# conroi/lcpc

Hardware: AMD Instinct MI355X
Metric: field-elements committed/sec (whole node), Ligero 2^26 coeffs (higher is better)
Workload: dtype u32 limbs (255-bit prime field Ft255, Montgomery form)

## Files before the change

### lcpc_amd/csrc/field_ln.h

```cpp
#pragma once
#include "field_dev.h"

namespace lcpc {

template <int NL, int W> constexpr u32 mod_limb(int k) {
  const int b = W * k, w = b / 32, sh = b % 32;
  const u64 lo = Mod<NL>::P[w], hi = (w + 1 < NL) ? Mod<NL>::P[w + 1] : 0;
  return (u32)(((lo | (hi << 32)) >> sh) & ((1u << W) - 1));
}
template <int FID> struct LnField;
template <> struct LnField<FT63> {
  static constexpr int FID = FT63, N = 3, W = 26, NL = 2, WAVES = 8, STRIDE = 4;
  static constexpr u32 limb(int k) { return mod_limb<NL, W>(k); }
};
template <> struct LnField<FT127> {
  static constexpr int FID = FT127, N = 5, W = 29, NL = 4, WAVES = 7, STRIDE = 8;
  static constexpr u32 limb(int k) { return mod_limb<NL, W>(k); }
};
template <> struct LnField<FT191> {
  static constexpr int FID = FT191, N = 7, W = 29, NL = 6, WAVES = 5, STRIDE = 8;
  static constexpr u32 limb(int k) { return mod_limb<NL, W>(k); }
};
template <> struct LnField<FT255> {
  static constexpr int FID = FT255, N = 9, W = 29, NL = 8, WAVES = 4, STRIDE = 12;
  static constexpr u32 limb(int k) { return mod_limb<NL, W>(k); }
};

#include "field_ln_gen.h"
#include "field_r29_gen.h"
#include "field_wmul_gen.h"

template <int N> struct LN {
  u32 v[N];
};

namespace ln {
constexpr int QOFF = 24;
constexpr int QBIAS = 40;

template <class FT> LCPC_DEV LN<FT::N> from_packed(const Fe<FT::NL>& a) {
  constexpr int N = FT::N, W = FT::W, NL = FT::NL;
  LN<N> r;
#pragma unroll
  for (int k = 0; k < N; k++) {
    const int b = W * k, w = b / 32, sh = b % 32;
    u32 x;
    if (sh == 0) x = a.v[w];
    else if (w + 1 < NL) x = __builtin_amdgcn_alignbit(a.v[w + 1], a.v[w], sh);
    else x = a.v[w] >> sh;
    r.v[k] = k + 1 < N ? (x & ((1u << W) - 1)) : x;
  }
  return r;
}
template <class FT> LCPC_DEV void to_packed(u32* out, const u32* l) {
  constexpr int N = FT::N, W = FT::W, NL = FT::NL;
#pragma unroll
  for (int w = 0; w < NL; w++) {
    u32 x = 0;
#pragma unroll
    for (int k = 0; k < N; k++) {
      const int off = W * k - 32 * w;
      if (off >= 0 && off < 32) x |= l[k] << off;
      else if (off < 0 && off > -32) x |= l[k] >> (-off);
    }
    out[w] = x;
  }
}
template <int N> LCPC_DEV LN<N> load_limbs(const u32* t) {
  LN<N> r;
  if constexpr (N == 3) {
    const uint2 a = *reinterpret_cast<const uint2*>(t);
    r.v[0] = a.x; r.v[1] = a.y; r.v[2] = t[2];
  } else {
    const uint4 a = *reinterpret_cast<const uint4*>(t);
    r.v[0] = a.x; r.v[1] = a.y; r.v[2] = a.z; r.v[3] = a.w;
    if constexpr (N == 5) r.v[4] = t[4];
    else if constexpr (N == 7) { const uint2 b = *reinterpret_cast<const uint2*>(t + 4); r.v[4] = b.x; r.v[5] = b.y; r.v[6] = t[6]; }
    else { const uint4 b = *reinterpret_cast<const uint4*>(t + 4); r.v[4] = b.x; r.v[5] = b.y; r.v[6] = b.z; r.v[7] = b.w; r.v[8] = t[8]; }
  }
  return r;
}
template <int N> LCPC_DEV LN<N> add(const LN<N>& a, const LN<N>& b) {
  LN<N> r;
#pragma unroll
  for (int k = 0; k < N; k++) r.v[k] = a.v[k] + b.v[k];
  return r;
}
template <int N> LCPC_DEV LN<N> sub(const LN<N>& a, const LN<N>& b) {
  LN<N> r;
#pragma unroll
  for (int k = 0; k < N; k++) r.v[k] = a.v[k] - b.v[k];
  return r;
}
template <class FT> LCPC_DEV void normalize(LN<FT::N>& a) {
#pragma unroll
  for (int k = 0; k + 1 < FT::N; k++) {
    a.v[k + 1] += (u32)((int32_t)a.v[k] >> FT::W);
    a.v[k] &= (1u << FT::W) - 1;
  }
}
template <class FT> LCPC_DEV u32 clamp_q(u32 top) {
  constexpr u32 PTOP1 = FT::limb(FT::N - 1) + 1;
  constexpr int SH = 31 - __builtin_clz(PTOP1);
  constexpr u32 MAGIC = (u32)((((u64)1 << (32 + SH)) + PTOP1 - 1) / PTOP1);
  static_assert((u64)64 * PTOP1 * PTOP1 < ((u64)1 << (32 + SH)), "magic division range");
  const u32 n = top + (u32)(QOFF * PTOP1 - QBIAS);
  return __umulhi(n, MAGIC) >> SH;
}
template <class FT> LCPC_DEV LN<FT::N> clamp_row(const u32* nqp, u32 q) { return load_limbs<FT::N>(nqp + q * FT::STRIDE); }
template <class FT> LCPC_DEV void clamp_apply(LN<FT::N>& a, const LN<FT::N>& nt) {
  int32_t c = 0;
#pragma unroll
  for (int k = 0; k + 1 < FT::N; k++) {
    const int32_t d = (int32_t)(a.v[k] + nt.v[k] + (u32)c);
    a.v[k] = (u32)d & ((1u << FT::W) - 1);
    c = d >> FT::W;
  }
  a.v[FT::N - 1] = a.v[FT::N - 1] + nt.v[FT::N - 1] + (u32)c;
}
template <class FT> LCPC_DEV LN<FT::N> mul(const LN<FT::N>& a, const LN<FT::N>& w) {
  LN<FT::N> r;
  if constexpr (FT::FID == FT63) ln_mul1s_ft63(a.v, w.v, r.v);
  else if constexpr (FT::FID == FT127) ln_mul1s_ft127(a.v, w.v, r.v);
  else if constexpr (FT::FID == FT191) ln_mul1s_ft191(a.v, w.v, r.v);
  else r29_mul1s(a.v, w.v, r.v);
  return r;
}
template <class FT> LCPC_DEV LN<FT::N> mul2(const LN<FT::N>& a, const LN<FT::N>& b0, const LN<FT::N>& b1) {
  static_assert(FT::FID == FT255, "the two-table multiply exists for Ft255 only");
  LN<FT::N> r = b1;
  r29_mul2s(a.v, b0.v, r.v);
  return r;
}
template <class FT> LCPC_DEV void mul2_pair(const LN<FT::N>& e, LN<FT::N>& b0, LN<FT::N>& b1) {
  static_assert(FT::FID == FT255, "the two-table multiply exists for Ft255 only");
#pragma unroll
  for (int t = 0; t < 2; t++) {
    LN<FT::N> kk;
#pragma unroll
    for (int z = 0; z < FT::N; z++) kk.v[z] = t ? R29_MUL2_KB[z] : R29_MUL2_KA[z];
    LN<FT::N> x = mul<FT>(kk, e);
    for (int it = 0; it < 2; it++) {
      if ((int32_t)x.v[FT::N - 1] < 0) {
#pragma unroll
        for (int z = 0; z < FT::N; z++) x.v[z] += FT::limb(z);
        normalize<FT>(x);
      }
    }
    (t ? b1 : b0) = x;
  }
}
template <class FT> constexpr bool has_mul_u = FT::N >= 5;
template <class FT> LCPC_DEV LN<FT::N> mul_u(const LN<FT::N>& a, const u32* wt) {
  static_assert(has_mul_u<FT>, "no shifted-multiples multiply for this field");
  LN<FT::N> r;
  if constexpr (FT::FID == FT127) wmul_u_ft127(a.v, wt, r.v);
  else if constexpr (FT::FID == FT191) wmul_u_ft191(a.v, wt, r.v);
  else {
    u32 np2[9];
#pragma unroll
    for (int j = 0; j < 9; j++) np2[j] = 0u - 2u * FT::limb(j);
    wmul_u(a.v, np2, wt, r.v);
  }
  return r;
}
template <class FT> struct LazyN {
  u64 c[2 * FT::N];
};
template <class FT> LCPC_DEV void lazy_zero(LazyN<FT>& a) {
#pragma unroll
  for (int k = 0; k < 2 * FT::N; k++) a.c[k] = 0;
}
template <class FT> LCPC_DEV void lazy_mac(LazyN<FT>& a, const LN<FT::N>& x, const LN<FT::N>& v) {
#pragma unroll
  for (int i = 0; i < FT::N; i++)
#pragma unroll
    for (int j = 0; j < FT::N; j++) a.c[i + j] += (u64)x.v[i] * v.v[j];
}
template <class FT> LCPC_DEV void lazy_normalize(LazyN<FT>& a) {
#pragma unroll
  for (int k = 0; k + 1 < 2 * FT::N; k++) {
    a.c[k + 1] += a.c[k] >> FT::W;
    a.c[k] &= (1u << FT::W) - 1;
  }
}
template <class FT> LCPC_DEV Fe<FT::NL> lazy_reduce(LazyN<FT>& a) {
  constexpr int N = FT::N, W = FT::W;
  constexpr u32 M = (1u << W) - 1;
  lazy_normalize<FT>(a);
  u32 m[N], r[N];
  u64 acc = 0;
#pragma unroll
  for (int k = 0; k < 2 * N; k++) {
    acc += a.c[k];
#pragma unroll
    for (int i = 0; i < N; i++) {
      const int j = k - i;
      if (i < k && j >= 1 && j < N) acc += (u64)m[i] * FT::limb(j);
    }
    if (k < N) {
      m[k] = (0u - (u32)acc) & M;
      acc += m[k];
      acc >>= W;
    } else {
      r[k - N] = (u32)acc & M;
      acc >>= W;
    }
  }
  u32 t[FT::NL];
  to_packed<FT>(t, r);
  return fe_reduce_once<FT::NL>(t);
}

LCPC_DEV void clamp(LN<9>& a, const u32* qp) {
  constexpr u32 M = (1u << 29) - 1;
  constexpr u32 PTOP1 = LnField<FT255>::limb(8) + 1;
  constexpr u64 MAGIC = (((u64)1 << 52) + PTOP1 - 1) / PTOP1;
  const u32 n = a.v[8] + (u32)(QOFF * PTOP1 - QBIAS);
  const u32 q = (u32)(((u64)n * MAGIC) >> 52);
  const u32* t = qp + q * 12;
  int32_t d[9];
#pragma unroll
  for (int k = 0; k < 9; k++) d[k] = (int32_t)(a.v[k] - t[k]);
#pragma unroll
  for (int k = 0; k < 8; k++) {
    d[k + 1] += d[k] >> 31;
    a.v[k] = (u32)d[k] & M;
  }
  a.v[8] = (u32)d[8];
}
LCPC_DEV Fe<8> to_packed_reduced(LN<9> a, const u32* qp) {
  clamp(a, qp);
  u32 t[8];
  to_packed<LnField<FT255>>(t, a.v);
  return fe_reduce_once<8>(t);
}
}

LCPC_DEV Fe<8> fe_mul_r29(const Fe<8>& a, const LN<9>& b) {
  const LN<9> x = ln::from_packed<LnField<FT255>>(a);
  u32 m[9], r[9];
  r29_columns(x.v, b.v, m, r);
  u32 t[8];
  ln::to_packed<LnField<FT255>>(t, r);
  return fe_reduce_once<8>(t);
}

LCPC_DEV Fe<8> fe_canon_r29(const Fe<8>& a) {
  using FT = LnField<FT255>;
  constexpr u32 M = (1u << 29) - 1;
  u32 x[9];
#pragma unroll
  for (int k = 0; k < 9; k++) {
    const int b = 29 * k - 5;
    u32 v;
    if (k == 0) v = (a.v[0] << 5);
    else {
      const int w = b / 32, sh = b % 32;
      if (sh == 0) v = a.v[w];
      else if (w + 1 < 8) v = __builtin_amdgcn_alignbit(a.v[w + 1], a.v[w], sh);
      else v = a.v[w] >> sh;
    }
    x[k] = v & M;
  }
  u32 m[9], r[9];
  u64 acc = 0;
#pragma unroll
  for (int k = 0; k < 17; k++) {
    if (k < 9) acc += x[k];
#pragma unroll
    for (int i = 0; i < 9; i++) {
      const int j = k - i;
      if (i < k && j >= 1 && j < 9) acc += (u64)m[i] * FT::limb(j);
    }
    if (k < 9) {
      m[k] = (0u - (u32)acc) & M;
      acc += m[k];
      acc >>= 29;
    } else {
      r[k - 9] = (u32)acc & M;
      acc >>= 29;
    }
  }
  r[8] = (u32)acc;
  u32 t[8];
  ln::to_packed<FT>(t, r);
  return fe_reduce_once<8>(t);
}

}
```

### lcpc_amd/csrc/gen/gen_r29_asm.py

```python
#!/usr/bin/env python3

N = 9


def block(terms, a_name, b_name):
    ins = []
    ops = []
    idx = {}

    def op(name, k):
        key = (name, k)
        if key not in idx:
            idx[key] = len(ops) + 1
            ops.append('"v"(%s[%d])' % (name, k) if name != "P" else '"s"(LnField<FT255>::limb(%d))' % k)
        return "%%%d" % idx[key]

    for i, j in terms:
        ins.append('"v_mad_u64_u32 %%0, vcc, %s, %s, %%0\\n\\t"' % (op(a_name, i), op(b_name, j)))
    return "    asm(" + "\n        ".join(ins) + '\n        : "+v"(acc) : ' + ", ".join(ops) + ' : "vcc");'


out = []
out.append("// GENERATED by lcpc_amd/csrc/gen/gen_r29_asm.py -- do not edit.  Column chains of fe_mul_r29 (see field_ln.h).")
out.append("// x: multiplicand limbs (u32[9]), b: twiddle limbs (u32[9]), m: quotient digits, r: result limbs")
out.append("LCPC_DEV void r29_columns(const u32* x, const u32* b, u32* m, u32* r) {")
out.append("  u64 acc = 0;")
for k in range(2 * N - 1):
    prod = [(i, k - i) for i in range(N) if 0 <= k - i < N]
    red = [(i, k - i) for i in range(N) if i < k and 1 <= k - i < N]
    out.append("  {  // column %d: %d products, %d reduction terms" % (k, len(prod), len(red)))
    out.append(block(prod, "x", "b"))
    if red:
        out.append(block(red, "m", "P"))
    if k < N:
        out.append("    m[%d] = (0u - (u32)acc) & 0x1fffffffu;" % k)
        out.append('    asm("v_mad_u64_u32 %%0, vcc, %%1, 1, %%0" : "+v"(acc) : "v"(m[%d]) : "vcc");   // + m_k * p_0 (= 1)' % k)
        out.append("    acc >>= 29;")
    else:
        out.append("    r[%d] = (u32)acc & 0x1fffffffu;" % (k - N))
        out.append("    acc >>= 29;")
    out.append("  }")
out.append("  r[8] = (u32)acc;")
out.append("}")


FT255_P = 0x663c799b6e4d2900fda9df04b9575969ef73c79086595f3002a4f20000000001
ACC = 126
PS = 92
acc = "v[%d:%d]" % (ACC, ACC + 1)
lo = "v%d" % ACC
R = lambda k: "%%%d" % k
X = lambda i: "%%%d" % (N + i)
B = lambda j: "%%%d" % (2 * N + j)
def mul1(signed):
    mad = "v_mad_i64_i32" if signed else "v_mad_u64_u32"
    shr = "v_ashrrev_i64" if signed else "v_lshrrev_b64"
    ins = []
    for j in range(1, N):
        pj = (FT255_P >> (29 * j)) & ((1 << 29) - 1)
        ins.append("s_mov_b32 s%d, 0x%x" % (PS + j - 1, ((-pj) & 0xffffffff) if signed else pj))
    first = True
    for k in range(2 * N - 1):
        for i in range(N):
            j = k - i
            if 0 <= j < N:
                ins.append("%s %s, vcc, %s, %s, %s" % (mad, acc, X(i), B(j), "0" if first else acc))
                first = False
        for i in range(N):
            j = k - i
            if i < k and 1 <= j < N:
                ins.append("%s %s, vcc, %s, s%d, %s" % (mad, acc, R(i), PS + j - 1, acc))
        if k < N and signed:
            ins.append("v_and_b32 %s, 0x1fffffff, %s" % (R(k), lo))
        elif k < N:
            ins.append("v_sub_u32 %s, 0, %s" % (R(k), lo))
            ins.append("v_and_b32 %s, 0x1fffffff, %s" % (R(k), R(k)))
            ins.append("v_mad_u64_u32 %s, vcc, %s, 1, %s" % (acc, R(k), acc))
        else:
            ins.append("v_and_b32 %s, 0x1fffffff, %s" % (R(k - N), lo))
        ins.append("%s %s, 29, %s" % (shr, acc, acc))
    ins.append("v_mov_b32 %s, %s" % (R(N - 1), lo))
    return ins


def emit(name, comment, ins):
    out.append("")
    out.append(comment)
    out.append("LCPC_DEV void %s(const u32* x, const u32* b, u32* r) {" % name)
    out.append("  asm(")
    for t in ins:
        out.append('      "%s\\n\\t"' % t)
    outs = ", ".join('"=&v"(r[%d])' % k for k in range(N))
    inps = ", ".join(['"v"(x[%d])' % i for i in range(N)] + ['"v"(b[%d])' % j for j in range(N)])
    clob = ", ".join(['"vcc"', '"v%d"' % ACC, '"v%d"' % (ACC + 1)] + ['"s%d"' % (PS + j) for j in range(N - 1)])
    out.append("      : %s\n      : %s\n      : %s);" % (outs, inps, clob))
    out.append("}")


out.append("")
out.append("// One-statement multiplies; they clobber v[%d:%d], s[%d:%d], vcc.  The asserts tie the literals to LnField<FT255>." % (ACC, ACC + 1, PS, PS + N - 2))
for j in range(1, N):
    out.append("static_assert(LnField<FT255>::limb(%d) == 0x%xu, \"gen_r29_asm.py modulus\");" % (j, (FT255_P >> (29 * j)) & ((1 << 29) - 1)))


ND2 = 5
def mul2():
    mad, shr = "v_mad_i64_i32", "v_ashrrev_i64"
    ins = []
    for j in range(1, N):
        pj = (FT255_P >> (29 * j)) & ((1 << 29) - 1)
        ins.append("s_mov_b32 s%d, 0x%x" % (PS + j - 1, (-pj) & 0xffffffff))
    first = True
    for k in range(N + ND2 - 1):
        for i in range(ND2):
            j = k - i
            if 0 <= j < N:
                ins.append("%s %s, vcc, %%[x%d], %%[a%d], %s" % (mad, acc, i, j, "0" if first else acc))
                first = False
        for i in range(N - ND2):
            j = k - i
            if 0 <= j < N:
                ins.append("%s %s, vcc, %%[x%d], %%[r%d], %s" % (mad, acc, ND2 + i, j, acc))
        for i in range(ND2):
            j = k - i
            if i < k and 1 <= j < N:
                ins.append("%s %s, vcc, %%[m%d], s%d, %s" % (mad, acc, i, PS + j - 1, acc))
        ins.append("v_and_b32 %%[%s], 0x1fffffff, %s" % ("m%d" % k if k < ND2 else "r%d" % (k - ND2), lo))
        ins.append("%s %s, 29, %s" % (shr, acc, acc))
    ins.append("v_mov_b32 %%[r%d], %s" % (N - 1, lo))
    return ins


def emit2(name, comment, ins):
    out.append("")
    out.append(comment)
    out.append("LCPC_DEV void %s(const u32* x, const u32* a, u32* r) {" % name)
    out.append("  u32 m0, m1, m2, m3, m4;")
    out.append("  asm(")
    for t in ins:
        out.append('      "%s\\n\\t"' % t)
    outs = ", ".join(['[r%d] "+v"(r[%d])' % (k, k) for k in range(N)] + ['[m%d] "=&v"(m%d)' % (k, k) for k in range(ND2)])
    inps = ", ".join(['[x%d] "v"(x[%d])' % (i, i) for i in range(N)] + ['[a%d] "v"(a[%d])' % (j, j) for j in range(N)])
    clob = ", ".join(['"vcc"', '"v%d"' % ACC, '"v%d"' % (ACC + 1)] + ['"s%d"' % (PS + j) for j in range(N - 1)])
    out.append("      : %s\n      : %s\n      : %s);" % (outs, inps, clob))
    out.append("}")


if __name__ == "__main__":
  emit("r29_mul1s", "// signed form (ln::mul<LnField<FT255>>): x limbs two's complement, |x_k| < 2^30, |value| < 16p; b as above.\n"
       "// r = x * b * 2^-261 in (-1.2p, 0.2p]: limbs 0..7 in [0, 2^29), top limb signed.", mul1(True))
  emit2("r29_mul2s", "// two-table form (ln::mul2<LnField<FT255>>): x limbs two's complement, |x_k| < 2^30; a = w c 2^145 mod p and, in r on entry,\n"
        "// b = w c 2^290 mod p, both in [0, p).  r = (XL a + XH b) 2^-145 == x w c in (-3.01p, 2.01p): limbs 0..7 in [0, 2^29), top limb signed.", mul2())
  for nm, e in (("R29_MUL2_KA", 145), ("R29_MUL2_KB", 290)):
      v = pow(2, e, FT255_P)
      out.append("constexpr u32 %s[9] = {%s};" % (nm, ", ".join("0x%xu" % ((v >> (29 * k)) & ((1 << 29) - 1)) for k in range(N))))
  print("\n".join(out))
```

### lcpc_amd/csrc/gen/gen_wmul_asm.py

```python
#!/usr/bin/env python3

FIELDS = {
    "ft255": (0x663c799b6e4d2900fda9df04b9575969ef73c79086595f3002a4f20000000001, 9, 29, 128),
    "ft63": (0x46d0760000000001, 3, 26, 64),
    "ft127": (0x6e754097ba20e0bf7f2bd90000000001, 5, 29, 72),
    "ft191": (0x453708aa3fbc8dda936888270ceecbcdd246820000000001, 7, 29, 96),
}


def params(field):
    P, N, W, VB = FIELDS[field]
    B = 1 << (W * (N - 1))
    ptop = P // B
    zmax = N * (1 << W) * (ptop + 1) // 2 + N + 1
    s1 = max(0, zmax.bit_length() - 31)
    if field == "ft255":
        s2 = 31
    else:
        s2 = 31
        while ((1 << (s1 + s2)) * B) // (2 * P) < (1 << 31):
            s2 += 1
        s2 -= 1
    MU = ((1 << (s1 + s2 - 1)) * B) // P
    assert MU < (1 << 31) and s2 < 64
    return P, N, W, VB, s1, s2, MU


def sreg_map(field):
    P, N, W, VB, s1, s2, MU = params(field)
    if field == "ft255":
        return (lambda t: 16 + t if t < 16 else (36 + t - 16 if t < 80 else 34)), 35, None
    return (lambda t: 36 + t), 36 + N * N, 36 + N * N + 1


def fixed_regs(field):
    VB = FIELDS[field][3]
    if field == "ft255":
        return VB - 2, VB - 4, VB - 6, VB - 10, VB - 8
    return VB - 2, VB - 4, VB - 6, VB - 2, VB - 7


def build(field):
    P, N, W, VB, s1, s2, MU = params(field)
    M = (1 << W) - 1
    sreg, S_MU, S_NP = sreg_map(field)
    A, Bv, C, T, Q = fixed_regs(field)
    acc = lambda r: "v[%d:%d]" % (r, r + 1)
    X = lambda j: "%%[x%d]" % j
    NP = (lambda k: "%%[n%d]" % k) if S_NP is None else (lambda k: "s%d" % (S_NP + k))
    R = lambda k: "%%[r%d]" % k
    Wl = lambda k, j: "s%d" % sreg(N * k + j)
    ins = []
    if field == "ft255":
        for blk in range(5):
            ins.append("s_load_dwordx16 s[%d:%d], %%[w], 0x%x" % (sreg(16 * blk), sreg(16 * blk) + 15, 64 * blk))
        ins.append("s_load_dword s%d, %%[w], 0x140" % sreg(80))
    else:
        t = 0
        while t < N * N:
            n = 16
            while n > N * N - t or (sreg(t) % min(n, 4)) != 0:
                n //= 2
            ins.append(("s_load_dword s%d" % sreg(t) if n == 1 else "s_load_dwordx%d s[%d:%d]" % (n, sreg(t), sreg(t) + n - 1)) + ", %%[w], 0x%x" % (4 * t))
            t += n
        for k in range(N):
            ins.append("s_mov_b32 s%d, 0x%x" % (S_NP + k, (-(((2 * P) >> (W * k)) & (M if k < N - 1 else (1 << 32) - 1))) & 0xffffffff))
    ins.append("s_mov_b32 s%d, 0x%x" % (S_MU, MU))
    ins.append("s_waitcnt lgkmcnt(0)")
    for k, reg in ((N - 1, C), (N - 2, Bv)):
        for j in range(N):
            ins.append("v_mad_i64_i32 %s, vcc, %s, %s, %s" % (acc(reg), X(j), Wl(k, j), "0" if j == 0 else acc(reg)))
    ins.append("v_ashrrev_i64 %s, %d, %s" % (acc(T), W, acc(Bv)))
    ins.append("v_add_co_u32 v%d, vcc, v%d, v%d" % (T, T, C))
    ins.append("v_addc_co_u32 v%d, vcc, v%d, v%d, vcc" % (T + 1, T + 1, C + 1))
    if s1:
        ins.append("v_ashrrev_i64 %s, %d, %s" % (acc(T), s1, acc(T)))
    ins.append("v_mad_i64_i32 %s, vcc, v%d, s%d, 0" % (acc(T), T, S_MU))
    ins.append("v_ashrrev_i64 %s, %d, %s" % (acc(T), s2, acc(T)))
    ins.append("v_add_u32 v%d, 1, v%d" % (Q, T))
    for k in range(N):
        if k < N - 2:
            for j in range(N):
                ins.append("v_mad_i64_i32 %s, vcc, %s, %s, %s" % (acc(A), X(j), Wl(k, j), "0" if (k == 0 and j == 0) else acc(A)))
        else:
            src = Bv if k == N - 2 else C
            ins.append("v_add_co_u32 v%d, vcc, v%d, v%d" % (A, A, src))
            ins.append("v_addc_co_u32 v%d, vcc, v%d, v%d, vcc" % (A + 1, A + 1, src + 1))
        ins.append("v_mad_i64_i32 %s, vcc, v%d, %s, %s" % (acc(A), Q, NP(k), acc(A)))
        if k < N - 1:
            ins.append("v_and_b32 %s, 0x%x, v%d" % (R(k), M, A))
            ins.append("v_ashrrev_i64 %s, %d, %s" % (acc(A), W, acc(A)))
        else:
            ins.append("v_mov_b32 %s, v%d" % (R(k), A))
    return ins


def emit(field):
    P, N, W, VB, s1, s2, MU = params(field)
    sreg, S_MU, S_NP = sreg_map(field)
    ins = build(field)
    A = fixed_regs(field)[0]
    T = min(fixed_regs(field))
    n_valu = sum(1 for i in ins if i.startswith("v_"))
    out = []
    if field == "ft255":
        out.append("// GENERATED by lcpc_amd/csrc/gen/gen_wmul_asm.py -- do not edit.  %d VALU instructions (%d mads) per multiply." % (n_valu, sum(1 for i in ins if i.startswith("v_mad"))))
        out.append("// np2: the nine limbs of -2p (signed); w: wave-uniform pointer to the 81 dwords of one twiddle's shifted multiples.")
        out.append("#define WMUL_MU 0x%xu" % MU)
        out.append("LCPC_DEV void wmul_u(const u32* x, const u32* np2, const u32* w, u32* r) {")
    else:
        out.append("")
        out.append("// %s: %d limbs of %d bits, %d VALU instructions (%d mads); w: wave-uniform pointer to the %d dwords t = %d k + j of one twiddle's" % (field, N, W, n_valu, sum(1 for i in ins if i.startswith("v_mad")), N * N, N))
        out.append("// shifted multiples.  Fixed registers v[%d:%d] (the top of the %d-VGPR budget of ntt_pass_lns_kernel<%s>)." % (T, A + 1, VB, field))
        out.append("LCPC_DEV void wmul_u_%s(const u32* x, const u32* w, u32* r) {" % field)
    out.append("  asm volatile(")
    for t in ins:
        out.append('      "%s\\n\\t"' % t)
    outs = ", ".join('[r%d] "=&v"(r[%d])' % (k, k) for k in range(N))
    inps = ['[x%d] "v"(x[%d])' % (j, j) for j in range(N)]
    if S_NP is None:
        inps += ['[n%d] "v"(np2[%d])' % (k, k) for k in range(N)]
    inps += ['[w] "s"(w)']
    sregs = ['"s%d"' % sreg(t) for t in range(N * N)] + ['"s%d"' % S_MU]
    if S_NP is not None:
        sregs = ['"s%d"' % sreg(t) for t in range(N * N)] + ['"s%d"' % S_MU] + ['"s%d"' % (S_NP + k) for k in range(N)]
    clob = ", ".join(['"vcc"'] + ['"v%d"' % v for v in range(T, A + 2)] + sregs + ['"memory"'])
    out.append("      : %s\n      : %s\n      : %s);" % (outs, ", ".join(inps), clob))
    out.append("}")
    return out


def main():
    out = emit("ft255")
    out.append("")
    out.append("// ---- the same multiply for the limb forms of field_ln.h (K1n, ntt_lns.hip); -2p and MU as scalar constants -------------------------")
    for f in ("ft63", "ft127", "ft191"):
        out += emit(f)
    print("\n".join(out))


if __name__ == "__main__":
    main()
```

### lcpc_amd/csrc/ntt_l9s.hip

```cpp
#include "kernels.h"
#include "ntt_ln_dev.h"

namespace lcpc {

namespace {

template <bool M2> struct Tw { LN<9> b0, b1; };
template <> struct Tw<false> { LN<9> b0; };
template <bool M2, u32 NV> LCPC_DEV Tw<M2> tw_get(const u32* blk, u32 period, u32 variant, u32 jl) {
  using FT = LnField<FT255>;
  Tw<M2> t;
  if constexpr (M2) {
    t.b0 = pack_get<FT, 2 * NV>(blk, period, variant, jl);
    t.b1 = pack_get<FT, 2 * NV>(blk, period, NV + variant, jl);
  } else {
    t.b0 = pack_get<FT, NV>(blk, period, variant, jl);
  }
  return t;
}
template <bool M2> LCPC_DEV LN<9> tw_mul(const LN<9>& x, const Tw<M2>& w) {
  if constexpr (M2) return ln::mul2<LnField<FT255>>(x, w.b0, w.b1);
  else return ln::mul<LnField<FT255>>(x, w.b0);
}

template <int S, int LTJ, bool FIRST, bool MID, bool NF, bool M2>
__global__ void __launch_bounds__(256, 4) ntt_pass_l9s_kernel(NttPassArgs a, const u32* __restrict__ pack, NttPackInfo pi) {
  using FT = LnField<FT255>;
  constexpr int NL = 8, LT = S + LTJ, LBT = LTJ;
  constexpr bool LAST = !FIRST;
  static_assert(LT == 10, "1024-element tiles: one radix-4 quad (two radix-2 pairs) per thread and round");
  static_assert(FIRST || (LTJ == 0 && S % 2 == 0), "the last pass works on contiguous tiles and ends with the trivial stages k-2, k-1");
  static_assert(NF || !M2, "the two-table multiply serves the pure / coset form only");
  using SH = Shape<S, LBT>;
  using SP = PureShape<S>;
  constexpr int RU = NF ? (FIRST ? SP::RU : -1) : SH::RU;
  constexpr int RC = NF && FIRST ? SP::RC : -1;
  constexpr bool SWZD = NF ? (LAST || SP::RU >= 0) : RU >= 0;
  auto SWZ = [](u32 e) -> u32 {
    if constexpr (NF && LAST) return e ^ (((e >> 4) & 3u) * 5u);
    else if constexpr (NF && FIRST && SWZD && LBT == 2) return e ^ ((((e >> 4) ^ (e >> 6)) & 3u) << 2);
    else if constexpr (SWZD) return e ^ ((e >> 4) & 15u);
    else return e;
  };
  extern __shared__ __attribute__((aligned(16))) u32 lds[];
  constexpr u32 T = 1u << LT;
  u32* nqp = lds + (size_t)T * 9;
  const u32 k = a.log_n;
  const u32 tiles_per_row = 1u << (k - LT);
  u64 row;
  u32 tile;
  if (FIRST && a.tile_group) {
    const u32 lg = a.tile_group;
    const u32 xcd = blockIdx.x & 7u;
    const u64 qq = blockIdx.x >> 3;
    const u32 sub = (u32)qq & ((1u << lg) - 1);
    const u64 q2 = qq >> lg;
    tile = (((u32)(q2 / a.n_rows) * 8u + xcd) << lg) | sub;
    row = q2 % a.n_rows;
  } else if (tiles_per_row >= 8) {
    const u32 xcd = blockIdx.x & 7u;
    const u64 qq = blockIdx.x >> 3;
    tile = (u32)(qq / a.n_rows) * 8u + xcd;
    row = qq % a.n_rows;
  } else {
    row = blockIdx.x / tiles_per_row;
    tile = blockIdx.x % tiles_per_row;
  }
  const u32 tid = threadIdx.x;
  mem_phase(true);
  const u32 lb = FIRST ? k - S : 0u;
  auto gindex = [&](u32 e) -> u32 {
    if constexpr (FIRST) return ((e >> LBT) << lb) | (tile << LTJ) | (e & ((1u << LBT) - 1));
    else return (tile << S) | e;
  };
  const bool canon = a.roots29c != nullptr && ((u32)row & a.canon_row_mask) == 0;
  for (u32 i = tid; i < 64 * 12; i += 256) nqp[i] = 0u - a.qp29[i];
  const u32* src = a.src + row * a.src_stride * NL;
  constexpr bool DIRECT = !(LAST && MID);
  LN<9> xin[4];
  if constexpr (LAST && MID) {
    const uint4* t4 = reinterpret_cast<const uint4*>(a.mid + (row << k) * 9 + (size_t)tile * (9 * T));
    uint4* l4 = reinterpret_cast<uint4*>(lds);
    if constexpr (SWZD) {
#pragma unroll
      for (u32 i = tid; i < 2 * T; i += 256) l4[(i & ~(T - 1)) | SWZ(i & (T - 1))] = t4[i];
#pragma unroll
      for (u32 i = tid; i < T / 4; i += 256) {
        const uint4 v = t4[2 * T + i];
        const u32 b = 8 * T + SWZ(4 * i);
        lds[b] = v.x; lds[b ^ 1u] = v.y; lds[b ^ 2u] = v.z; lds[b ^ 3u] = v.w;
      }
    } else {
#pragma unroll
    for (u32 i = tid; i < 9 * T / 4; i += 256) l4[i] = t4[i];
    }
  } else {
#pragma unroll
  for (u32 it = 0; it < 4; it++) {
    const u32 e = tid + 256u * it;
    const u32 g = gindex(e);
    Fe<NL> v;
    if constexpr (FIRST) {
      v = (g < a.n_valid && row * a.src_stride + g < a.n_src_total) ? fe_load<NL>(src + (size_t)g * NL) : fe_zero<NL>();
      if (a.copy_dst != nullptr && g < a.n_valid) fe_store<NL>(a.copy_dst + (row * a.src_stride + g) * NL, v);
    } else {
      v = fe_load<NL>(src + (size_t)g * NL);
    }
    xin[it] = ln::from_packed<FT>(v);
  }
  __builtin_amdgcn_sched_barrier(0);
  }
  const u32* cls_pack = pack + (size_t)(FIRST != NF ? tile : 0u) * pi.class_words;
  const bool blk0_tile = (FIRST || tile == 0) && a.blk0_gone == 0;
  LN<9> k32;
#pragma unroll
  for (int i = 0; i < 9; i++) k32.v[i] = i == 0 ? 32u : 0u;
  const bool zero_hi = FIRST && a.n_valid <= (1ull << (k - 1));
  if constexpr (!DIRECT) __syncthreads();

  if constexpr (SH::U0 == 1) {
    constexpr u32 half = 1u << (S - 1 + LBT);
    const u32* blk = cls_pack + pi.round_off[0];
#pragma unroll
    for (u32 pp = 0; pp < 2; pp++) {
      const u32 e1 = tid + 256u * pp;
      const Tw<M2> w = NF ? tw_get<M2, 2>(blk, 1u << (S - 1), canon ? 1u : 0u, e1 >> LBT) : tw_get<M2, 2>(blk, SH::period2, canon ? 1u : 0u, e1);
      const LN<9> x = DIRECT ? xin[pp] : planes_get<FT>(lds, T, SWZ(e1));
      if (pp == 0) mem_phase(false);
      const bool cvs = NF && canon && SH::NR4 <= 1;
      if (zero_hi) {
        if constexpr (DIRECT) planes_put<FT>(lds, T, SWZ(e1), cvs ? ln::mul<FT>(x, k32) : x);
        planes_put<FT>(lds, T, SWZ(e1 + half), tw_mul<M2>(x, w));
      } else {
        const LN<9> y = DIRECT ? xin[pp + 2] : planes_get<FT>(lds, T, SWZ(e1 + half));
        LN<9> sum = ln::add(x, y);
        ln::normalize<FT>(sum);
        planes_put<FT>(lds, T, SWZ(e1), cvs ? ln::mul<FT>(sum, k32) : sum);
        planes_put<FT>(lds, T, SWZ(e1 + half), tw_mul<M2>(ln::sub(x, y), w));
      }
    }
    mem_phase(true);
    __syncthreads();
  }

  const u32 q = tid;
  if constexpr (NF && LAST) {
#pragma unroll
    for (int r = 0; r < 5; r++) {
      const int hb = 9 - 2 * r;
      const u32 D = 1u << (hb - 1);
      const u32 m = q >> (hb - 1);
      const u32 e0 = (m << (hb + 1)) | (q & (D - 1));
      const bool from_regs = DIRECT && r == 0;
      LN<9> x0 = from_regs ? xin[0] : planes_get<FT>(lds, T, SWZ(e0));
      const LN<9> x1 = from_regs ? xin[1] : planes_get<FT>(lds, T, SWZ(e0 + D));
      const LN<9> x2 = from_regs ? xin[2] : planes_get<FT>(lds, T, SWZ(e0 + 2 * D)), x3 = from_regs ? xin[3] : planes_get<FT>(lds, T, SWZ(e0 + 3 * D));
      LN<9> p1, p2, p3;
      if (r < 2) {
        const u32 sb = r == 0 ? 0u : (u32)__builtin_amdgcn_readfirstlane(tid >> 6);
        const u32* wu = cls_pack + pi.u_off + ((u32)r * 4 + sb) * (3 * U_SLOT<FT>);
        mem_phase(false);
        if (!from_regs) ln::clamp_apply<FT>(x0, ln::clamp_row<FT>(nqp, ln::clamp_q<FT>(x0.v[8])));
        p2 = ln::mul_u<FT>(x2, wu + U_SLOT<FT>);
        p1 = ln::mul_u<FT>(x1, wu);
        p3 = ln::mul_u<FT>(x3, wu + 2 * U_SLOT<FT>);
      } else {
        const u32* blk = cls_pack + pi.round_off[r];
        const Tw<M2> w1 = tw_get<M2, 3>(blk, coset_sets(r), 0, m), w2 = tw_get<M2, 3>(blk, coset_sets(r), 1, m);
        const Tw<M2> w3 = tw_get<M2, 3>(blk, coset_sets(r), 2, m);
        mem_phase(false);
        ln::clamp_apply<FT>(x0, ln::clamp_row<FT>(nqp, ln::clamp_q<FT>(x0.v[8])));
        p2 = tw_mul<M2>(x2, w2);
        p1 = tw_mul<M2>(x1, w1);
        p3 = tw_mul<M2>(x3, w3);
      }
      const LN<9> s02 = ln::add(x0, p2), d02 = ln::sub(x0, p2), s13 = ln::add(p1, p3);
      LN<9> y0 = ln::add(s02, s13), y1 = ln::sub(s02, s13);
      if (r < 4) ln::normalize<FT>(y0);
      const LN<9> t = ln::mul_u<FT>(ln::sub(p1, p3), a.wq_w);
      LN<9> y2 = ln::add(d02, t), y3 = ln::sub(d02, t);
      if (r == 0) { ln::normalize<FT>(y1); ln::normalize<FT>(y2); ln::normalize<FT>(y3); }
      mem_phase(true);
      if (r < 4) {
        planes_put<FT>(lds, T, SWZ(e0), y0);
        planes_put<FT>(lds, T, SWZ(e0 + D), y1);
        planes_put<FT>(lds, T, SWZ(e0 + 2 * D), y2);
        planes_put<FT>(lds, T, SWZ(e0 + 3 * D), y3);
        __syncthreads();
      } else {
        u32* dstq = a.dst + row * a.dst_stride * NL + (size_t)((tile << S) | e0) * NL;
        clamp_store<FT, true>(dstq, y0, nqp);
        clamp_store<FT, true>(dstq + (size_t)1 * NL, y1, nqp);
        clamp_store<FT, true>(dstq + (size_t)2 * NL, y2, nqp);
        clamp_store<FT, true>(dstq + (size_t)3 * NL, y3, nqp);
      }
    }
    return;
  }
#pragma unroll
  for (int r = 0; r < SH::NR4; r++) {
    const int u = SH::U0 + 2 * r, hb = S - u - 1;
    const bool last_two = LAST && (r == SH::NR4 - 1);
    const bool triv = NF && FIRST && (r == SH::NR4 - 1);
    const u32 lp = q & ((1u << LBT) - 1), j = q >> LBT;
    const u32 i0 = ((j >> (hb - 1)) << (hb + 1)) | (j & ((1u << (hb - 1)) - 1));
    const u32 e0 = (i0 << LBT) | lp;
    constexpr u32 one = 1u;
    const u32 dq = one << (hb - 1 + LBT);
    const u32 period = NF ? one << (hb - 1) : one << (hb - 1 + LBT);
    const u32 jl = NF ? j & (period - 1) : q & (period - 1);
    const u32* blk = cls_pack + pi.round_off[SH::U0 + r];
    if (triv) {
      const bool fr = DIRECT && SH::U0 == 0 && r == 0;
      const LN<9> x0 = fr ? xin[0] : planes_get<FT>(lds, T, SWZ(e0)), x1 = fr ? xin[1] : planes_get<FT>(lds, T, SWZ(e0 + dq));
      const LN<9> x2 = fr ? xin[2] : planes_get<FT>(lds, T, SWZ(e0 + 2 * dq)), x3 = fr ? xin[3] : planes_get<FT>(lds, T, SWZ(e0 + 3 * dq));
      mem_phase(false);
      const LN<9> b0 = ln::add(x0, x2), b1 = ln::add(x1, x3);
      LN<9> c0 = ln::add(b0, b1), c1 = ln::sub(b0, b1);
      const LN<9> b2 = ln::sub(x0, x2);
      const LN<9> t = ln::mul_u<FT>(ln::sub(x1, x3), a.wq_w);
      LN<9> c2 = ln::add(b2, t), c3 = ln::sub(b2, t);
      if constexpr (!MID && SH::NR4 >= 1) {
        if (RC < 0 && SH::U0 == 0 && canon) {
          ln::normalize<FT>(c0); ln::normalize<FT>(c1); ln::normalize<FT>(c2); ln::normalize<FT>(c3);
          c0 = ln::mul<FT>(c0, k32); c1 = ln::mul<FT>(c1, k32); c2 = ln::mul<FT>(c2, k32); c3 = ln::mul<FT>(c3, k32);
        }
        if constexpr (SH::U0 == 0 && SH::NR4 == 1) __syncthreads();
        mem_phase(true);
        u32* dstq = a.dst + row * a.dst_stride * NL;
        clamp_store<FT, false>(dstq + (size_t)gindex(e0) * NL, c0, nqp);
        clamp_store<FT, false>(dstq + (size_t)gindex(e0 + dq) * NL, c1, nqp);
        clamp_store<FT, false>(dstq + (size_t)gindex(e0 + 2 * dq) * NL, c2, nqp);
        clamp_store<FT, false>(dstq + (size_t)gindex(e0 + 3 * dq) * NL, c3, nqp);
        return;
      }
      ln::normalize<FT>(c1); ln::normalize<FT>(c2); ln::normalize<FT>(c3);
      if (RC < 0 && SH::U0 == 0 && canon) {
        ln::normalize<FT>(c0);
        c0 = ln::mul<FT>(c0, k32); c1 = ln::mul<FT>(c1, k32); c2 = ln::mul<FT>(c2, k32); c3 = ln::mul<FT>(c3, k32);
      } else if (fr) {
        ln::normalize<FT>(c0);
      } else {
        ln::clamp_apply<FT>(c0, ln::clamp_row<FT>(nqp, ln::clamp_q<FT>(c0.v[8])));
      }
      planes_put<FT>(lds, T, SWZ(e0), c0);
      planes_put<FT>(lds, T, SWZ(e0 + dq), c1);
      planes_put<FT>(lds, T, SWZ(e0 + 2 * dq), c2);
      planes_put<FT>(lds, T, SWZ(e0 + 3 * dq), c3);
      mem_phase(true);
      __syncthreads();
      continue;
    }
    if constexpr (RU >= 0) {
      if (r >= RU && !last_two) {
        const u32 wv = __builtin_amdgcn_readfirstlane(tid >> 6);
        const u32 qu = NF ? (((((tid & 63u) >> LBT) << 2) | wv) << LBT) | (tid & ((1u << LBT) - 1)) : ((tid & 63u) << 2) | wv;
        const u32 lpu = qu & ((1u << LBT) - 1), ju = qu >> LBT;
        const u32 iu = ((ju >> (hb - 1)) << (hb + 1)) | (ju & ((1u << (hb - 1)) - 1));
        const u32 eu = (iu << LBT) | lpu;
        const u32* wu = cls_pack + pi.u_off + ((r - RU) * 4 + wv) * (3 * U_SLOT<FT>);
        const LN<9> x0 = planes_get<FT>(lds, T, SWZ(eu)), x1 = planes_get<FT>(lds, T, SWZ(eu + dq));
        const LN<9> x2 = planes_get<FT>(lds, T, SWZ(eu + 2 * dq)), x3 = planes_get<FT>(lds, T, SWZ(eu + 3 * dq));
        mem_phase(false);
        const LN<9> b0 = ln::add(x0, x2), b1 = ln::add(x1, x3);
        LN<9> c0 = ln::add(b0, b1);
        ln::clamp_apply<FT>(c0, ln::clamp_row<FT>(nqp, ln::clamp_q<FT>(c0.v[8])));
        planes_put<FT>(lds, T, SWZ(eu), c0);
        LN<9> d1 = ln::sub(b0, b1);
        ln::normalize<FT>(d1);
        planes_put<FT>(lds, T, SWZ(eu + dq), ln::mul_u<FT>(d1, wu + 2 * U_SLOT<FT>));
        const LN<9> b2 = ln::mul_u<FT>(ln::sub(x0, x2), wu);
        const LN<9> b3 = ln::mul_u<FT>(ln::sub(x1, x3), wu + U_SLOT<FT>);
        LN<9> c2 = ln::add(b2, b3);
        if constexpr (NF || (FIRST && MID)) ln::clamp_apply<FT>(c2, ln::clamp_row<FT>(nqp, ln::clamp_q<FT>(c2.v[8])));
        else ln::normalize<FT>(c2);
        planes_put<FT>(lds, T, SWZ(eu + 2 * dq), c2);
        planes_put<FT>(lds, T, SWZ(eu + 3 * dq), ln::mul_u<FT>(ln::sub(b2, b3), wu + 2 * U_SLOT<FT>));
        mem_phase(true);
        __syncthreads();
        continue;
      }
    }
    if (u == 0 && zero_hi) {
      const u32 vb = canon ? 3u : 0u;
      const Tw<M2> w0 = tw_get<M2, 6>(blk, period, vb + 0, jl), w3 = tw_get<M2, 6>(blk, period, vb + 1, jl), w2 = tw_get<M2, 6>(blk, period, vb + 2, jl);
      mem_phase(false);
      const bool cv0 = NF && canon && r == RC;
      if (a.n_valid <= (1ull << (k - 2))) {
        const LN<9> x0 = DIRECT ? xin[0] : planes_get<FT>(lds, T, SWZ(e0));
        if constexpr (DIRECT) planes_put<FT>(lds, T, SWZ(e0), cv0 ? ln::mul<FT>(x0, k32) : x0);
        planes_put<FT>(lds, T, SWZ(e0 + dq), tw_mul<M2>(x0, w2));
        planes_put<FT>(lds, T, SWZ(e0 + 2 * dq), tw_mul<M2>(x0, w0));
        planes_put<FT>(lds, T, SWZ(e0 + 3 * dq), tw_mul<M2>(x0, w3));
      } else {
        const LN<9> x0 = DIRECT ? xin[0] : planes_get<FT>(lds, T, SWZ(e0)), x1 = DIRECT ? xin[1] : planes_get<FT>(lds, T, SWZ(e0 + dq));
        LN<9> c0 = ln::add(x0, x1);
        ln::normalize<FT>(c0);
        planes_put<FT>(lds, T, SWZ(e0), cv0 ? ln::mul<FT>(c0, k32) : c0);
        planes_put<FT>(lds, T, SWZ(e0 + dq), tw_mul<M2>(ln::sub(x0, x1), w2));
        const LN<9> t = ln::mul_u<FT>(x1, a.wq_w);
        planes_put<FT>(lds, T, SWZ(e0 + 2 * dq), tw_mul<M2>(ln::add(x0, t), w0));
        planes_put<FT>(lds, T, SWZ(e0 + 3 * dq), tw_mul<M2>(ln::sub(x0, t), w3));
      }
      mem_phase(true);
      __syncthreads();
      continue;
    }
    const bool from_regs = DIRECT && SH::U0 == 0 && r == 0;
    const LN<9> x0 = from_regs ? xin[0] : planes_get<FT>(lds, T, SWZ(e0)), x1 = from_regs ? xin[1] : planes_get<FT>(lds, T, SWZ(e0 + dq));
    const LN<9> x2 = from_regs ? xin[2] : planes_get<FT>(lds, T, SWZ(e0 + 2 * dq)), x3 = from_regs ? xin[3] : planes_get<FT>(lds, T, SWZ(e0 + 3 * dq));
    mem_phase(false);
    const LN<9> b0 = ln::add(x0, x2), b1 = ln::add(x1, x3);
    LN<9> c0 = ln::add(b0, b1);
    if (last_two) {
      LN<9> c1 = ln::sub(b0, b1);
      const LN<9> b2 = ln::sub(x0, x2);
      const LN<9> b3 = ln::mul_u<FT>(ln::sub(x1, x3), a.wq_w);
      LN<9> c2 = ln::add(b2, b3);
      LN<9> c3 = ln::sub(b2, b3);
      mem_phase(true);
      u32* dstq = a.dst + row * a.dst_stride * NL + (size_t)((tile << S) | e0) * NL;
      clamp_store<FT, true>(dstq, c0, nqp);
      clamp_store<FT, true>(dstq + (size_t)1 * NL, c1, nqp);
      clamp_store<FT, true>(dstq + (size_t)2 * NL, c2, nqp);
      clamp_store<FT, true>(dstq + (size_t)3 * NL, c3, nqp);
      return;
    } else {
      if (from_regs) ln::normalize<FT>(c0);
      else ln::clamp_apply<FT>(c0, ln::clamp_row<FT>(nqp, ln::clamp_q<FT>(c0.v[8])));
      planes_put<FT>(lds, T, SWZ(e0), c0);
      const bool blk0c = NF ? canon && q < dq : canon && blk0_tile && q < period && (RU < 0 || r < RU);
      if constexpr (NF ? RC >= 0 : RU >= 1) {
        if (r == (NF ? RC : RU - 1) && blk0c) {
          planes_put<FT>(lds, T, SWZ(e0), ln::mul<FT>(c0, k32));
        }
      }
      const u32 vb = blk0c ? 3u : 0u;
      if constexpr (M2) {
        const Tw<M2> w2 = tw_get<M2, 6>(blk, period, vb + 2, jl), w0 = tw_get<M2, 6>(blk, period, vb + 0, jl);
        const LN<9> d1 = ln::sub(b0, b1);
        const LN<9> d13 = ln::sub(x1, x3), e2 = ln::sub(x0, x2);
        planes_put<FT>(lds, T, SWZ(e0 + dq), tw_mul<M2>(d1, w2));
        __builtin_amdgcn_sched_barrier(0);
        const Tw<M2> w3 = tw_get<M2, 6>(blk, period, vb + 1, jl);
        const LN<9> t = ln::mul_u<FT>(d13, a.wq_w);
        planes_put<FT>(lds, T, SWZ(e0 + 2 * dq), tw_mul<M2>(ln::add(e2, t), w0));
        planes_put<FT>(lds, T, SWZ(e0 + 3 * dq), tw_mul<M2>(ln::sub(e2, t), w3));
      } else {
      const Tw<M2> w0 = tw_get<M2, 6>(blk, period, vb + 0, jl), w3 = tw_get<M2, 6>(blk, period, vb + 1, jl);
      const Tw<M2> w2 = tw_get<M2, 6>(blk, period, vb + 2, jl);
      const LN<9> d1 = ln::sub(b0, b1);
      planes_put<FT>(lds, T, SWZ(e0 + dq), tw_mul<M2>(d1, w2));
      const LN<9> t = ln::mul_u<FT>(ln::sub(x1, x3), a.wq_w);
      const LN<9> e2 = ln::sub(x0, x2);
      planes_put<FT>(lds, T, SWZ(e0 + 2 * dq), tw_mul<M2>(ln::add(e2, t), w0));
      planes_put<FT>(lds, T, SWZ(e0 + 3 * dq), tw_mul<M2>(ln::sub(e2, t), w3));
      }
    }
    mem_phase(true);
    __syncthreads();
  }

  if constexpr (FIRST && MID) {
    u32* mrow = a.mid + (row << k) * 9;
#pragma unroll
    for (u32 e = tid; e < T; e += 256) {
      const u32 e2 = (tile << LTJ) | (e & ((1u << LBT) - 1));
      u32* t = mrow + (size_t)(e >> LBT) * (9 * T);
      const LN<9> x = planes_get<FT>(lds, T, SWZ(e));
      *reinterpret_cast<uint4*>(t + (size_t)e2 * 4) = make_uint4(x.v[0], x.v[1], x.v[2], x.v[3]);
      *reinterpret_cast<uint4*>(t + (size_t)(T + e2) * 4) = make_uint4(x.v[4], x.v[5], x.v[6], x.v[7]);
      t[(size_t)8 * T + e2] = x.v[8];
    }
    return;
  }
  if constexpr (FIRST) {
  u32* dst = a.dst + row * a.dst_stride * NL;
#pragma unroll
  for (u32 e = tid; e < T; e += 256) {
    const u32 g = gindex(e);
    LN<9> x = planes_get<FT>(lds, T, SWZ(e));
    ln::clamp_apply<FT>(x, ln::clamp_row<FT>(nqp, ln::clamp_q<FT>(x.v[8])));
    u32 w[8];
    ln::to_packed<FT>(w, x.v);
    Fe<NL> v;
#pragma unroll
    for (int i = 0; i < 8; i++) v.v[i] = w[i];
    fe_store<NL>(dst + (size_t)g * NL, v);
  }
  }
}

template <int S, int LTJ, bool FIRST, bool MID, bool NF, bool M2>
hipError_t launch_tm(const NttPassArgs& a, const u32* pack, const NttPackInfo& pi, hipStream_t st) {
  constexpr int LT = S + LTJ;
  const u64 tiles = ((u64)1 << (a.log_n - LT)) * a.n_rows;
  const size_t lds_bytes = (((size_t)1 << LT) * 9 + 64 * LnField<FT255>::STRIDE) * 4;
  hipError_t e = hipFuncSetAttribute(reinterpret_cast<const void*>(&ntt_pass_l9s_kernel<S, LTJ, FIRST, MID, NF, M2>),
                                     hipFuncAttributeMaxDynamicSharedMemorySize, (int)lds_bytes);
  if (e != hipSuccess) return e;
  hipLaunchKernelGGL((ntt_pass_l9s_kernel<S, LTJ, FIRST, MID, NF, M2>), dim3((unsigned)tiles), dim3(256), lds_bytes, st, a, pack, pi);
  return hipGetLastError();
}
template <int S, int LTJ, bool FIRST>
hipError_t launch_t(const NttPassArgs& a, const u32* pack, const NttPackInfo& pi, hipStream_t st) {
  if (pi.mul2) {
    if constexpr (ntt_l9s_mul2_supported(S, FIRST)) { if (a.form) return a.mid ? launch_tm<S, LTJ, FIRST, true, true, true>(a, pack, pi, st) : launch_tm<S, LTJ, FIRST, false, true, true>(a, pack, pi, st); }
    return hipErrorInvalidValue;
  }
  if (a.form) return a.mid ? launch_tm<S, LTJ, FIRST, true, true, false>(a, pack, pi, st) : launch_tm<S, LTJ, FIRST, false, true, false>(a, pack, pi, st);
  return a.mid ? launch_tm<S, LTJ, FIRST, true, false, false>(a, pack, pi, st) : launch_tm<S, LTJ, FIRST, false, false, false>(a, pack, pi, st);
}

}

bool ntt_l9s3_supported(uint32_t log_n) { return log_n >= 21 && log_n <= 26; }

bool ntt_l9s_supported(uint32_t log_n, uint32_t n_passes, int log_tile) { return n_passes == 2 && log_tile == 10 && log_n >= 11 && log_n <= 20; }

#define L9S_FIRST_CASES(X) X(1) X(2) X(3) X(4) X(5) X(6) X(7) X(8) X(9) X(10)

hipError_t launch_ntt_pass_l9s(const NttPassArgs& a, bool first, const uint32_t* pack, const NttPackInfo& pi, hipStream_t st) {
  if (!first) {
    if (a.s != 10 || a.log_tj != 0 || a.t0 + a.s != a.log_n) return hipErrorInvalidValue;
    if (a.mont_prefix) return hipErrorInvalidValue;
    return launch_t<10, 0, false>(a, pack, pi, st);
  }
  if (a.t0 != 0 || a.s + a.log_tj != 10 || (a.s + 10 != a.log_n && a.s + 20 != a.log_n)) return hipErrorInvalidValue;
  if (a.form && a.s + 10 != a.log_n) return hipErrorInvalidValue;
  if (a.tile_group && ((1u << (a.log_n - 10)) >> a.tile_group) < 8) return hipErrorInvalidValue;
  switch (a.s) {
#define X(SV) case SV: return launch_t<SV, 10 - SV, true>(a, pack, pi, st);
    L9S_FIRST_CASES(X)
#undef X
  }
  return hipErrorInvalidValue;
}

}
```

### lcpc_amd/csrc/ntt_ln_dev.h

```cpp
#pragma once
#include "field_ln.h"

namespace lcpc {

template <int S, int LBT> struct Shape {
  static constexpr int U0 = S & 1;
  static constexpr int NR4 = S / 2;
  static constexpr u32 period2 = 1u << (S - 1 + LBT);
  static constexpr u32 period4(int r) { return 1u << (S - U0 - 2 * r - 2 + LBT); }
  static constexpr int RU = NR4 >= 4 ? 3 : -1;
  static constexpr int NRU = RU < 0 ? 0 : NR4 - RU;
};
template <int S> struct PureShape {
  static constexpr int U0 = S & 1;
  static constexpr int NR4 = S / 2;
  static constexpr u32 sets(int r) { return 1u << (S - U0 - 2 * r - 2); }
  static constexpr int RU = NR4 >= 3 ? NR4 - 2 : -1;
  static constexpr int RC = NR4 >= 3 ? NR4 - 3 : (NR4 == 2 ? 0 : -1);
};
constexpr u32 coset_sets(int r) { return 1u << (2 * r); }

template <class FT> constexpr u32 U_SLOT = (FT::N * FT::N + 31) & ~31u;
template <class FT> constexpr u32 U_ALIGN = FT::N == 9 ? 4u : 16u;

template <class FT, class C = u32> LCPC_DEV LN<FT::N> planes_get(const u32* base, C cnt, u32 e) {
  constexpr int N = FT::N;
  LN<N> r;
  if constexpr (N == 3) {
    const uint2 a = *reinterpret_cast<const uint2*>(base + (size_t)e * 2);
    r.v[0] = a.x; r.v[1] = a.y; r.v[2] = base[(size_t)cnt * 2 + e];
  } else {
    const uint4 a = *reinterpret_cast<const uint4*>(base + (size_t)e * 4);
    r.v[0] = a.x; r.v[1] = a.y; r.v[2] = a.z; r.v[3] = a.w;
    if constexpr (N == 5) {
      r.v[4] = base[(size_t)cnt * 4 + e];
    } else if constexpr (N == 7) {
      const uint2 b = *reinterpret_cast<const uint2*>(base + (size_t)cnt * 4 + (size_t)e * 2);
      r.v[4] = b.x; r.v[5] = b.y; r.v[6] = base[(size_t)cnt * 6 + e];
    } else {
      const uint4 b = *reinterpret_cast<const uint4*>(base + ((size_t)cnt + e) * 4);
      r.v[4] = b.x; r.v[5] = b.y; r.v[6] = b.z; r.v[7] = b.w; r.v[8] = base[(size_t)cnt * 8 + e];
    }
  }
  return r;
}
template <class FT, class C = u32> LCPC_DEV void planes_put(u32* base, C cnt, u32 e, const LN<FT::N>& x) {
  constexpr int N = FT::N;
  if constexpr (N == 3) {
    *reinterpret_cast<uint2*>(base + (size_t)e * 2) = make_uint2(x.v[0], x.v[1]);
    base[(size_t)cnt * 2 + e] = x.v[2];
  } else {
    *reinterpret_cast<uint4*>(base + (size_t)e * 4) = make_uint4(x.v[0], x.v[1], x.v[2], x.v[3]);
    if constexpr (N == 5) {
      base[(size_t)cnt * 4 + e] = x.v[4];
    } else if constexpr (N == 7) {
      *reinterpret_cast<uint2*>(base + (size_t)cnt * 4 + (size_t)e * 2) = make_uint2(x.v[4], x.v[5]);
      base[(size_t)cnt * 6 + e] = x.v[6];
    } else {
      *reinterpret_cast<uint4*>(base + ((size_t)cnt + e) * 4) = make_uint4(x.v[4], x.v[5], x.v[6], x.v[7]);
      base[(size_t)cnt * 8 + e] = x.v[8];
    }
  }
}

template <class FT, bool REDUCE> LCPC_DEV void clamp_store(u32* dst, LN<FT::N> x, const u32* nqp) {
  constexpr int N = FT::N, NL = FT::NL;
  ln::clamp_apply<FT>(x, ln::clamp_row<FT>(nqp, ln::clamp_q<FT>(x.v[N - 1])));
  u32 w[NL];
  ln::to_packed<FT>(w, x.v);
  Fe<NL> v;
#pragma unroll
  for (int i = 0; i < NL; i++) v.v[i] = w[i];
  if constexpr (REDUCE) {
    if (__any((int)(x.v[N - 1] >= FT::limb(N - 1)))) v = fe_reduce_once<NL>(w);
  }
  fe_store<NL>(dst, v);
}

template <class FT> LCPC_DEV LN<FT::N> tab_entry(const u32* tab, u32 idx) {
  if constexpr (FT::STRIDE == 12) {
    return ln::load_limbs<FT::N>(tab + (size_t)idx * 12);
  } else {
    LN<FT::N> t;
#pragma unroll
    for (int k = 0; k < FT::N; k++) t.v[k] = tab[(size_t)idx * FT::STRIDE + k];
    return t;
  }
}

template <class FT, u32 NV> LCPC_DEV LN<FT::N> pack_get(const u32* blk, u32 period, u32 variant, u32 jl) {
  if constexpr (FT::N == 9) {
    const char* base = reinterpret_cast<const char*>(blk);
    const uint4 a = *reinterpret_cast<const uint4*>(base + (((variant * 2 + 0) * period + jl) << 4));
    const uint4 b = *reinterpret_cast<const uint4*>(base + (((variant * 2 + 1) * period + jl) << 4));
    const u32 c = *reinterpret_cast<const u32*>(base + ((NV * 2 * period * 4 + variant * period + jl) << 2));
    LN<9> t;
    t.v[0] = a.x; t.v[1] = a.y; t.v[2] = a.z; t.v[3] = a.w; t.v[4] = b.x; t.v[5] = b.y; t.v[6] = b.z; t.v[7] = b.w; t.v[8] = c;
    return t;
  } else {
    return planes_get<FT>(blk, NV * period, variant * period + jl);
  }
}
template <class FT, u32 NV> LCPC_DEV void pack_put(u32* blk, u32 period, u32 variant, u32 jl, const LN<FT::N>& x) {
  if constexpr (FT::N == 9) {
    *reinterpret_cast<uint4*>(blk + ((size_t)(variant * 2 + 0) * period + jl) * 4) = make_uint4(x.v[0], x.v[1], x.v[2], x.v[3]);
    *reinterpret_cast<uint4*>(blk + ((size_t)(variant * 2 + 1) * period + jl) * 4) = make_uint4(x.v[4], x.v[5], x.v[6], x.v[7]);
    blk[(size_t)NV * 2 * period * 4 + (size_t)variant * period + jl] = x.v[8];
  } else {
    planes_put<FT>(blk, NV * period, variant * period + jl, x);
  }
}

}
```

Before: 7.799 billion.

## Use uniform-base addressing and a short-tail multiply in the Ft255 NTT kernel

Global pointers are forced wave-uniform with readfirstlane (ubase) and per-lane accesses become 32-bit byte offsets (lane_at), so the compiler can keep the base in scalar registers and use SGPR-based addressing instead of 64-bit per-lane address arithmetic. Twiddle fetches are split into a uniform variant and a lane-varying variant to fit this scheme. The generated multiplies gain a short-tail variant that drops the final shift and carry steps of the top limb, cutting a few VALU instructions per call. A guard on log_n > 26 is added so the 32-bit offsets cannot overflow, and this limits supported sizes.

```diff
diff --git a/lcpc_amd/csrc/field_ln.h b/lcpc_amd/csrc/field_ln.h
--- a/lcpc_amd/csrc/field_ln.h
+++ b/lcpc_amd/csrc/field_ln.h
@@ -164,6 +164,15 @@
   }
   return r;
 }
+template <class FT> LCPC_DEV LN<FT::N> mul_us(const LN<FT::N>& a, const u32* wt) {
+  static_assert(FT::FID == FT255, "the short-tail statement exists for Ft255 only");
+  LN<FT::N> r;
+  u32 np2[9];
+#pragma unroll
+  for (int j = 0; j < 9; j++) np2[j] = 0u - 2u * FT::limb(j);
+  wmul_us(a.v, np2, wt, r.v);
+  return r;
+}
 template <class FT> struct LazyN {
   u64 c[2 * FT::N];
 };
diff --git a/lcpc_amd/csrc/gen/gen_r29_asm.py b/lcpc_amd/csrc/gen/gen_r29_asm.py
--- a/lcpc_amd/csrc/gen/gen_r29_asm.py
+++ b/lcpc_amd/csrc/gen/gen_r29_asm.py
@@ -104,7 +104,7 @@
 
 
 ND2 = 5
-def mul2():
+def mul2(short_tail=False):
     mad, shr = "v_mad_i64_i32", "v_ashrrev_i64"
     ins = []
     for j in range(1, N):
@@ -126,6 +126,9 @@
             if i < k and 1 <= j < N:
                 ins.append("%s %s, vcc, %%[m%d], s%d, %s" % (mad, acc, i, PS + j - 1, acc))
         ins.append("v_and_b32 %%[%s], 0x1fffffff, %s" % ("m%d" % k if k < ND2 else "r%d" % (k - ND2), lo))
+        if short_tail and k == N + ND2 - 2:
+            ins.append("v_alignbit_b32 %%[r%d], v%d, %s, 29" % (N - 1, ACC + 1, lo))
+            return ins
         ins.append("%s %s, 29, %s" % (shr, acc, acc))
     ins.append("v_mov_b32 %%[r%d], %s" % (N - 1, lo))
     return ins
@@ -150,7 +153,7 @@
   emit("r29_mul1s", "// signed form (ln::mul<LnField<FT255>>): x limbs two's complement, |x_k| < 2^30, |value| < 16p; b as above.\n"
        "// r = x * b * 2^-261 in (-1.2p, 0.2p]: limbs 0..7 in [0, 2^29), top limb signed.", mul1(True))
   emit2("r29_mul2s", "// two-table form (ln::mul2<LnField<FT255>>): x limbs two's complement, |x_k| < 2^30; a = w c 2^145 mod p and, in r on entry,\n"
-        "// b = w c 2^290 mod p, both in [0, p).  r = (XL a + XH b) 2^-145 == x w c in (-3.01p, 2.01p): limbs 0..7 in [0, 2^29), top limb signed.", mul2())
+        "// b = w c 2^290 mod p, both in [0, p).  r = (XL a + XH b) 2^-145 == x w c in (-3.01p, 2.01p): limbs 0..7 in [0, 2^29), top limb signed.", mul2(short_tail=True))
   for nm, e in (("R29_MUL2_KA", 145), ("R29_MUL2_KB", 290)):
       v = pow(2, e, FT255_P)
       out.append("constexpr u32 %s[9] = {%s};" % (nm, ", ".join("0x%xu" % ((v >> (29 * k)) & ((1 << 29) - 1)) for k in range(N))))
diff --git a/lcpc_amd/csrc/gen/gen_wmul_asm.py b/lcpc_amd/csrc/gen/gen_wmul_asm.py
--- a/lcpc_amd/csrc/gen/gen_wmul_asm.py
+++ b/lcpc_amd/csrc/gen/gen_wmul_asm.py
@@ -40,7 +40,7 @@
     return VB - 2, VB - 4, VB - 6, VB - 2, VB - 7
 
 
-def build(field):
+def build(field, short_tail=False):
     P, N, W, VB, s1, s2, MU = params(field)
     M = (1 << W) - 1
     sreg, S_MU, S_NP = sreg_map(field)
@@ -82,6 +82,10 @@
         if k < N - 2:
             for j in range(N):
                 ins.append("v_mad_i64_i32 %s, vcc, %s, %s, %s" % (acc(A), X(j), Wl(k, j), "0" if (k == 0 and j == 0) else acc(A)))
+        elif k == N - 1 and short_tail:
+            ins.append("v_mul_lo_u32 v%d, v%d, %s" % (T, Q, NP(k)))
+            ins.append("v_add3_u32 %s, v%d, v%d, v%d" % (R(k), A, C, T))
+            break
         else:
             src = Bv if k == N - 2 else C
             ins.append("v_add_co_u32 v%d, vcc, v%d, v%d" % (A, A, src))
@@ -95,15 +99,19 @@
     return ins
 
 
-def emit(field):
+def emit(field, short_tail=False):
     P, N, W, VB, s1, s2, MU = params(field)
     sreg, S_MU, S_NP = sreg_map(field)
-    ins = build(field)
+    ins = build(field, short_tail)
     A = fixed_regs(field)[0]
     T = min(fixed_regs(field))
     n_valu = sum(1 for i in ins if i.startswith("v_"))
     out = []
-    if field == "ft255":
+    if field == "ft255" and short_tail:
+        out.append("")
+        out.append("// the same multiply with the short tail (build(field, short_tail=True)): %d VALU instructions (%d mads), bit for bit wmul_u's result." % (n_valu, sum(1 for i in ins if i.startswith("v_mad"))))
+        out.append("LCPC_DEV void wmul_us(const u32* x, const u32* np2, const u32* w, u32* r) {")
+    elif field == "ft255":
         out.append("// GENERATED by lcpc_amd/csrc/gen/gen_wmul_asm.py -- do not edit.  %d VALU instructions (%d mads) per multiply." % (n_valu, sum(1 for i in ins if i.startswith("v_mad"))))
         out.append("// np2: the nine limbs of -2p (signed); w: wave-uniform pointer to the 81 dwords of one twiddle's shifted multiples.")
         out.append("#define WMUL_MU 0x%xu" % MU)
@@ -131,7 +139,7 @@
 
 
 def main():
-    out = emit("ft255")
+    out = emit("ft255") + emit("ft255", short_tail=True)
     out.append("")
     out.append("// ---- the same multiply for the limb forms of field_ln.h (K1n, ntt_lns.hip); -2p and MU as scalar constants -------------------------")
     for f in ("ft63", "ft127", "ft191"):
diff --git a/lcpc_amd/csrc/ntt_l9s.hip b/lcpc_amd/csrc/ntt_l9s.hip
--- a/lcpc_amd/csrc/ntt_l9s.hip
+++ b/lcpc_amd/csrc/ntt_l9s.hip
@@ -7,14 +7,13 @@
 
 template <bool M2> struct Tw { LN<9> b0, b1; };
 template <> struct Tw<false> { LN<9> b0; };
-template <bool M2, u32 NV> LCPC_DEV Tw<M2> tw_get(const u32* blk, u32 period, u32 variant, u32 jl) {
-  using FT = LnField<FT255>;
+template <bool M2, u32 NV> LCPC_DEV Tw<M2> tw_get(const u32* blk, u32 period, u32 uv, u32 lv, u32 jl) {
   Tw<M2> t;
   if constexpr (M2) {
-    t.b0 = pack_get<FT, 2 * NV>(blk, period, variant, jl);
-    t.b1 = pack_get<FT, 2 * NV>(blk, period, NV + variant, jl);
+    t.b0 = pack_get_u<2 * NV>(blk, period, uv, lv, jl);
+    t.b1 = pack_get_u<2 * NV>(blk, period, NV + uv, lv, jl);
   } else {
-    t.b0 = pack_get<FT, NV>(blk, period, variant, jl);
+    t.b0 = pack_get_u<NV>(blk, period, uv, lv, jl);
   }
   return t;
 }
@@ -74,12 +73,14 @@
     else return (tile << S) | e;
   };
   const bool canon = a.roots29c != nullptr && ((u32)row & a.canon_row_mask) == 0;
-  for (u32 i = tid; i < 64 * 12; i += 256) nqp[i] = 0u - a.qp29[i];
-  const u32* src = a.src + row * a.src_stride * NL;
+  for (u32 i = tid; i < 64 * 12; i += 256) nqp[i] = 0u - *lane_at(ubase(a.qp29), i * 4u);
+  const u64 src_row = row * a.src_stride;
+  const u32* src = ubase(a.src + (src_row + (FIRST ? 0u : (u64)tile << S)) * NL);
+  const u32 n_val = (u32)(a.n_valid < ((u64)1 << k) ? a.n_valid : (u64)1 << k);
   constexpr bool DIRECT = !(LAST && MID);
   LN<9> xin[4];
   if constexpr (LAST && MID) {
-    const uint4* t4 = reinterpret_cast<const uint4*>(a.mid + (row << k) * 9 + (size_t)tile * (9 * T));
+    const uint4* t4 = reinterpret_cast<const uint4*>(ubase(a.mid + (row << k) * 9 + (size_t)tile * (9 * T)));
     uint4* l4 = reinterpret_cast<uint4*>(lds);
     if constexpr (SWZD) {
 #pragma unroll
@@ -98,24 +99,26 @@
 #pragma unroll
   for (u32 it = 0; it < 4; it++) {
     const u32 e = tid + 256u * it;
-    const u32 g = gindex(e);
     Fe<NL> v;
     if constexpr (FIRST) {
-      v = (g < a.n_valid && row * a.src_stride + g < a.n_src_total) ? fe_load<NL>(src + (size_t)g * NL) : fe_zero<NL>();
-      if (a.copy_dst != nullptr && g < a.n_valid) fe_store<NL>(a.copy_dst + (row * a.src_stride + g) * NL, v);
+      const u32 g = gindex(e);
+      const u64 left = a.n_src_total > src_row ? a.n_src_total - src_row : 0;
+      const u32 n_src = left < n_val ? (u32)left : n_val;
+      v = g < n_src ? fe_load<NL>(lane_at(src, g * (NL * 4u))) : fe_zero<NL>();
+      if (a.copy_dst != nullptr && g < n_val) fe_store<NL>(lane_at(ubase(a.copy_dst + src_row * NL), g * (NL * 4u)), v);
     } else {
-      v = fe_load<NL>(src + (size_t)g * NL);
+      v = fe_load<NL>(lane_at(ubase(src + 256u * it * NL), tid * (NL * 4u)));
     }
     xin[it] = ln::from_packed<FT>(v);
   }
   __builtin_amdgcn_sched_barrier(0);
   }
-  const u32* cls_pack = pack + (size_t)(FIRST != NF ? tile : 0u) * pi.class_words;
+  const u32* cls_pack = ubase(pack + (size_t)(FIRST != NF ? tile : 0u) * pi.class_words);
   const bool blk0_tile = (FIRST || tile == 0) && a.blk0_gone == 0;
   LN<9> k32;
 #pragma unroll
   for (int i = 0; i < 9; i++) k32.v[i] = i == 0 ? 32u : 0u;
-  const bool zero_hi = FIRST && a.n_valid <= (1ull << (k - 1));
+  const bool zero_hi = FIRST && n_val <= (1u << (k - 1));
   if constexpr (!DIRECT) __syncthreads();
 
   if constexpr (SH::U0 == 1) {
@@ -124,7 +127,7 @@
 #pragma unroll
     for (u32 pp = 0; pp < 2; pp++) {
       const u32 e1 = tid + 256u * pp;
-      const Tw<M2> w = NF ? tw_get<M2, 2>(blk, 1u << (S - 1), canon ? 1u : 0u, e1 >> LBT) : tw_get<M2, 2>(blk, SH::period2, canon ? 1u : 0u, e1);
+      const Tw<M2> w = NF ? tw_get<M2, 2>(blk, 1u << (S - 1), 0, canon ? 1u : 0u, e1 >> LBT) : tw_get<M2, 2>(blk, SH::period2, 0, canon ? 1u : 0u, e1);
       const LN<9> x = DIRECT ? xin[pp] : planes_get<FT>(lds, T, SWZ(e1));
       if (pp == 0) mem_phase(false);
       const bool cvs = NF && canon && SH::NR4 <= 1;
@@ -161,13 +164,13 @@
         const u32* wu = cls_pack + pi.u_off + ((u32)r * 4 + sb) * (3 * U_SLOT<FT>);
         mem_phase(false);
         if (!from_regs) ln::clamp_apply<FT>(x0, ln::clamp_row<FT>(nqp, ln::clamp_q<FT>(x0.v[8])));
-        p2 = ln::mul_u<FT>(x2, wu + U_SLOT<FT>);
-        p1 = ln::mul_u<FT>(x1, wu);
-        p3 = ln::mul_u<FT>(x3, wu + 2 * U_SLOT<FT>);
+        p2 = ln::mul_us<FT>(x2, wu + U_SLOT<FT>);
+        p1 = ln::mul_us<FT>(x1, wu);
+        p3 = ln::mul_us<FT>(x3, wu + 2 * U_SLOT<FT>);
       } else {
         const u32* blk = cls_pack + pi.round_off[r];
-        const Tw<M2> w1 = tw_get<M2, 3>(blk, coset_sets(r), 0, m), w2 = tw_get<M2, 3>(blk, coset_sets(r), 1, m);
-        const Tw<M2> w3 = tw_get<M2, 3>(blk, coset_sets(r), 2, m);
+        const Tw<M2> w1 = tw_get<M2, 3>(blk, coset_sets(r), 0, 0, m), w2 = tw_get<M2, 3>(blk, coset_sets(r), 1, 0, m);
+        const Tw<M2> w3 = tw_get<M2, 3>(blk, coset_sets(r), 2, 0, m);
         mem_phase(false);
         ln::clamp_apply<FT>(x0, ln::clamp_row<FT>(nqp, ln::clamp_q<FT>(x0.v[8])));
         p2 = tw_mul<M2>(x2, w2);
@@ -177,7 +180,7 @@
       const LN<9> s02 = ln::add(x0, p2), d02 = ln::sub(x0, p2), s13 = ln::add(p1, p3);
       LN<9> y0 = ln::add(s02, s13), y1 = ln::sub(s02, s13);
       if (r < 4) ln::normalize<FT>(y0);
-      const LN<9> t = ln::mul_u<FT>(ln::sub(p1, p3), a.wq_w);
+      const LN<9> t = ln::mul_us<FT>(ln::sub(p1, p3), a.wq_w);
       LN<9> y2 = ln::add(d02, t), y3 = ln::sub(d02, t);
       if (r == 0) { ln::normalize<FT>(y1); ln::normalize<FT>(y2); ln::normalize<FT>(y3); }
       mem_phase(true);
@@ -188,11 +191,11 @@
         planes_put<FT>(lds, T, SWZ(e0 + 3 * D), y3);
         __syncthreads();
       } else {
-        u32* dstq = a.dst + row * a.dst_stride * NL + (size_t)((tile << S) | e0) * NL;
-        clamp_store<FT, true>(dstq, y0, nqp);
-        clamp_store<FT, true>(dstq + (size_t)1 * NL, y1, nqp);
-        clamp_store<FT, true>(dstq + (size_t)2 * NL, y2, nqp);
-        clamp_store<FT, true>(dstq + (size_t)3 * NL, y3, nqp);
+        u32* dstq = a.dst + (row * a.dst_stride + ((u64)tile << S)) * NL;
+        clamp_store<FT, true>(lane_at(ubase(dstq + 0 * NL), e0 * (NL * 4u)), y0, nqp);
+        clamp_store<FT, true>(lane_at(ubase(dstq + 1 * NL), e0 * (NL * 4u)), y1, nqp);
+        clamp_store<FT, true>(lane_at(ubase(dstq + 2 * NL), e0 * (NL * 4u)), y2, nqp);
+        clamp_store<FT, true>(lane_at(ubase(dstq + 3 * NL), e0 * (NL * 4u)), y3, nqp);
       }
     }
     return;
@@ -218,7 +221,7 @@
       const LN<9> b0 = ln::add(x0, x2), b1 = ln::add(x1, x3);
       LN<9> c0 = ln::add(b0, b1), c1 = ln::sub(b0, b1);
       const LN<9> b2 = ln::sub(x0, x2);
-      const LN<9> t = ln::mul_u<FT>(ln::sub(x1, x3), a.wq_w);
+      const LN<9> t = ln::mul_us<FT>(ln::sub(x1, x3), a.wq_w);
       LN<9> c2 = ln::add(b2, t), c3 = ln::sub(b2, t);
       if constexpr (!MID && SH::NR4 >= 1) {
         if (RC < 0 && SH::U0 == 0 && canon) {
@@ -227,11 +230,11 @@
         }
         if constexpr (SH::U0 == 0 && SH::NR4 == 1) __syncthreads();
         mem_phase(true);
-        u32* dstq = a.dst + row * a.dst_stride * NL;
-        clamp_store<FT, false>(dstq + (size_t)gindex(e0) * NL, c0, nqp);
-        clamp_store<FT, false>(dstq + (size_t)gindex(e0 + dq) * NL, c1, nqp);
-        clamp_store<FT, false>(dstq + (size_t)gindex(e0 + 2 * dq) * NL, c2, nqp);
-        clamp_store<FT, false>(dstq + (size_t)gindex(e0 + 3 * dq) * NL, c3, nqp);
+        u32* dstq = ubase(a.dst + row * a.dst_stride * NL);
+        clamp_store<FT, false>(lane_at(dstq, gindex(e0) * (NL * 4u)), c0, nqp);
+        clamp_store<FT, false>(lane_at(dstq, gindex(e0 + dq) * (NL * 4u)), c1, nqp);
+        clamp_store<FT, false>(lane_at(dstq, gindex(e0 + 2 * dq) * (NL * 4u)), c2, nqp);
+        clamp_store<FT, false>(lane_at(dstq, gindex(e0 + 3 * dq) * (NL * 4u)), c3, nqp);
         return;
       }
       ln::normalize<FT>(c1); ln::normalize<FT>(c2); ln::normalize<FT>(c3);
@@ -268,14 +271,14 @@
         planes_put<FT>(lds, T, SWZ(eu), c0);
         LN<9> d1 = ln::sub(b0, b1);
         ln::normalize<FT>(d1);
-        planes_put<FT>(lds, T, SWZ(eu + dq), ln::mul_u<FT>(d1, wu + 2 * U_SLOT<FT>));
-        const LN<9> b2 = ln::mul_u<FT>(ln::sub(x0, x2), wu);
-        const LN<9> b3 = ln::mul_u<FT>(ln::sub(x1, x3), wu + U_SLOT<FT>);
+        planes_put<FT>(lds, T, SWZ(eu + dq), ln::mul_us<FT>(d1, wu + 2 * U_SLOT<FT>));
+        const LN<9> b2 = ln::mul_us<FT>(ln::sub(x0, x2), wu);
+        const LN<9> b3 = ln::mul_us<FT>(ln::sub(x1, x3), wu + U_SLOT<FT>);
         LN<9> c2 = ln::add(b2, b3);
         if constexpr (NF || (FIRST && MID)) ln::clamp_apply<FT>(c2, ln::clamp_row<FT>(nqp, ln::clamp_q<FT>(c2.v[8])));
         else ln::normalize<FT>(c2);
         planes_put<FT>(lds, T, SWZ(eu + 2 * dq), c2);
-        planes_put<FT>(lds, T, SWZ(eu + 3 * dq), ln::mul_u<FT>(ln::sub(b2, b3), wu + 2 * U_SLOT<FT>));
+        planes_put<FT>(lds, T, SWZ(eu + 3 * dq), ln::mul_us<FT>(ln::sub(b2, b3), wu + 2 * U_SLOT<FT>));
         mem_phase(true);
         __syncthreads();
         continue;
@@ -283,10 +286,10 @@
     }
     if (u == 0 && zero_hi) {
       const u32 vb = canon ? 3u : 0u;
-      const Tw<M2> w0 = tw_get<M2, 6>(blk, period, vb + 0, jl), w3 = tw_get<M2, 6>(blk, period, vb + 1, jl), w2 = tw_get<M2, 6>(blk, period, vb + 2, jl);
+      const Tw<M2> w0 = tw_get<M2, 6>(blk, period, 0, vb, jl), w3 = tw_get<M2, 6>(blk, period, 1, vb, jl), w2 = tw_get<M2, 6>(blk, period, 2, vb, jl);
       mem_phase(false);
       const bool cv0 = NF && canon && r == RC;
-      if (a.n_valid <= (1ull << (k - 2))) {
+      if (n_val <= (1u << (k - 2))) {
         const LN<9> x0 = DIRECT ? xin[0] : planes_get<FT>(lds, T, SWZ(e0));
         if constexpr (DIRECT) planes_put<FT>(lds, T, SWZ(e0), cv0 ? ln::mul<FT>(x0, k32) : x0);
         planes_put<FT>(lds, T, SWZ(e0 + dq), tw_mul<M2>(x0, w2));
@@ -298,7 +301,7 @@
         ln::normalize<FT>(c0);
         planes_put<FT>(lds, T, SWZ(e0), cv0 ? ln::mul<FT>(c0, k32) : c0);
         planes_put<FT>(lds, T, SWZ(e0 + dq), tw_mul<M2>(ln::sub(x0, x1), w2));
-        const LN<9> t = ln::mul_u<FT>(x1, a.wq_w);
+        const LN<9> t = ln::mul_us<FT>(x1, a.wq_w);
         planes_put<FT>(lds, T, SWZ(e0 + 2 * dq), tw_mul<M2>(ln::add(x0, t), w0));
         planes_put<FT>(lds, T, SWZ(e0 + 3 * dq), tw_mul<M2>(ln::sub(x0, t), w3));
       }
@@ -315,15 +318,15 @@
     if (last_two) {
       LN<9> c1 = ln::sub(b0, b1);
       const LN<9> b2 = ln::sub(x0, x2);
-      const LN<9> b3 = ln::mul_u<FT>(ln::sub(x1, x3), a.wq_w);
+      const LN<9> b3 = ln::mul_us<FT>(ln::sub(x1, x3), a.wq_w);
       LN<9> c2 = ln::add(b2, b3);
       LN<9> c3 = ln::sub(b2, b3);
       mem_phase(true);
-      u32* dstq = a.dst + row * a.dst_stride * NL + (size_t)((tile << S) | e0) * NL;
-      clamp_store<FT, true>(dstq, c0, nqp);
-      clamp_store<FT, true>(dstq + (size_t)1 * NL, c1, nqp);
-      clamp_store<FT, true>(dstq + (size_t)2 * NL, c2, nqp);
-      clamp_store<FT, true>(dstq + (size_t)3 * NL, c3, nqp);
+      u32* dstq = a.dst + (row * a.dst_stride + ((u64)tile << S)) * NL;
+      clamp_store<FT, true>(lane_at(ubase(dstq + 0 * NL), e0 * (NL * 4u)), c0, nqp);
+      clamp_store<FT, true>(lane_at(ubase(dstq + 1 * NL), e0 * (NL * 4u)), c1, nqp);
+      clamp_store<FT, true>(lane_at(ubase(dstq + 2 * NL), e0 * (NL * 4u)), c2, nqp);
+      clamp_store<FT, true>(lane_at(ubase(dstq + 3 * NL), e0 * (NL * 4u)), c3, nqp);
       return;
     } else {
       if (from_regs) ln::normalize<FT>(c0);
@@ -337,21 +340,21 @@
       }
       const u32 vb = blk0c ? 3u : 0u;
       if constexpr (M2) {
-        const Tw<M2> w2 = tw_get<M2, 6>(blk, period, vb + 2, jl), w0 = tw_get<M2, 6>(blk, period, vb + 0, jl);
+        const Tw<M2> w2 = tw_get<M2, 6>(blk, period, 2, vb, jl), w0 = tw_get<M2, 6>(blk, period, 0, vb, jl);
         const LN<9> d1 = ln::sub(b0, b1);
         const LN<9> d13 = ln::sub(x1, x3), e2 = ln::sub(x0, x2);
         planes_put<FT>(lds, T, SWZ(e0 + dq), tw_mul<M2>(d1, w2));
         __builtin_amdgcn_sched_barrier(0);
-        const Tw<M2> w3 = tw_get<M2, 6>(blk, period, vb + 1, jl);
-        const LN<9> t = ln::mul_u<FT>(d13, a.wq_w);
+        const Tw<M2> w3 = tw_get<M2, 6>(blk, period, 1, vb, jl);
+        const LN<9> t = ln::mul_us<FT>(d13, a.wq_w);
         planes_put<FT>(lds, T, SWZ(e0 + 2 * dq), tw_mul<M2>(ln::add(e2, t), w0));
         planes_put<FT>(lds, T, SWZ(e0 + 3 * dq), tw_mul<M2>(ln::sub(e2, t), w3));
       } else {
-      const Tw<M2> w0 = tw_get<M2, 6>(blk, period, vb + 0, jl), w3 = tw_get<M2, 6>(blk, period, vb + 1, jl);
-      const Tw<M2> w2 = tw_get<M2, 6>(blk, period, vb + 2, jl);
+      const Tw<M2> w0 = tw_get<M2, 6>(blk, period, 0, vb, jl), w3 = tw_get<M2, 6>(blk, period, 1, vb, jl);
+      const Tw<M2> w2 = tw_get<M2, 6>(blk, period, 2, vb, jl);
       const LN<9> d1 = ln::sub(b0, b1);
       planes_put<FT>(lds, T, SWZ(e0 + dq), tw_mul<M2>(d1, w2));
-      const LN<9> t = ln::mul_u<FT>(ln::sub(x1, x3), a.wq_w);
+      const LN<9> t = ln::mul_us<FT>(ln::sub(x1, x3), a.wq_w);
       const LN<9> e2 = ln::sub(x0, x2);
       planes_put<FT>(lds, T, SWZ(e0 + 2 * dq), tw_mul<M2>(ln::add(e2, t), w0));
       planes_put<FT>(lds, T, SWZ(e0 + 3 * dq), tw_mul<M2>(ln::sub(e2, t), w3));
@@ -362,22 +365,26 @@
   }
 
   if constexpr (FIRST && MID) {
-    u32* mrow = a.mid + (row << k) * 9;
-#pragma unroll
-    for (u32 e = tid; e < T; e += 256) {
+    u32* mrow = ubase(a.mid + (row << k) * 9);
+    u32 tid_st = tid;
+    asm volatile("" : "+v"(tid_st));
+#pragma unroll
+    for (u32 e = tid_st; e < T; e += 256) {
       const u32 e2 = (tile << LTJ) | (e & ((1u << LBT) - 1));
-      u32* t = mrow + (size_t)(e >> LBT) * (9 * T);
+      const u32 t = (e >> LBT) * (9 * T * 4u);
       const LN<9> x = planes_get<FT>(lds, T, SWZ(e));
-      *reinterpret_cast<uint4*>(t + (size_t)e2 * 4) = make_uint4(x.v[0], x.v[1], x.v[2], x.v[3]);
-      *reinterpret_cast<uint4*>(t + (size_t)(T + e2) * 4) = make_uint4(x.v[4], x.v[5], x.v[6], x.v[7]);
-      t[(size_t)8 * T + e2] = x.v[8];
+      *reinterpret_cast<uint4*>(lane_at(mrow, t + e2 * 16u)) = make_uint4(x.v[0], x.v[1], x.v[2], x.v[3]);
+      *reinterpret_cast<uint4*>(lane_at(mrow, t + (T + e2) * 16u)) = make_uint4(x.v[4], x.v[5], x.v[6], x.v[7]);
+      *lane_at(mrow, t + (8 * T + e2) * 4u) = x.v[8];
     }
     return;
   }
   if constexpr (FIRST) {
-  u32* dst = a.dst + row * a.dst_stride * NL;
-#pragma unroll
-  for (u32 e = tid; e < T; e += 256) {
+  u32* dst = ubase(a.dst + row * a.dst_stride * NL);
+  u32 tid_st = tid;
+  asm volatile("" : "+v"(tid_st));
+#pragma unroll
+  for (u32 e = tid_st; e < T; e += 256) {
     const u32 g = gindex(e);
     LN<9> x = planes_get<FT>(lds, T, SWZ(e));
     ln::clamp_apply<FT>(x, ln::clamp_row<FT>(nqp, ln::clamp_q<FT>(x.v[8])));
@@ -386,7 +393,7 @@
     Fe<NL> v;
 #pragma unroll
     for (int i = 0; i < 8; i++) v.v[i] = w[i];
-    fe_store<NL>(dst + (size_t)g * NL, v);
+    fe_store<NL>(lane_at(dst, g * (NL * 4u)), v);
   }
   }
 }
@@ -428,6 +435,7 @@
   }
   if (a.t0 != 0 || a.s + a.log_tj != 10 || (a.s + 10 != a.log_n && a.s + 20 != a.log_n)) return hipErrorInvalidValue;
   if (a.form && a.s + 10 != a.log_n) return hipErrorInvalidValue;
+  if (a.log_n > 26) return hipErrorInvalidValue;
   if (a.tile_group && ((1u << (a.log_n - 10)) >> a.tile_group) < 8) return hipErrorInvalidValue;
   switch (a.s) {
 #define X(SV) case SV: return launch_t<SV, 10 - SV, true>(a, pack, pi, st);
diff --git a/lcpc_amd/csrc/ntt_ln_dev.h b/lcpc_amd/csrc/ntt_ln_dev.h
--- a/lcpc_amd/csrc/ntt_ln_dev.h
+++ b/lcpc_amd/csrc/ntt_ln_dev.h
@@ -22,6 +22,15 @@
 
 template <class FT> constexpr u32 U_SLOT = (FT::N * FT::N + 31) & ~31u;
 template <class FT> constexpr u32 U_ALIGN = FT::N == 9 ? 4u : 16u;
+
+template <class T> LCPC_DEV T* ubase(T* p) {
+  const u64 v = reinterpret_cast<u64>(p);
+  const u32 lo = __builtin_amdgcn_readfirstlane((u32)v), hi = __builtin_amdgcn_readfirstlane((u32)(v >> 32));
+  typedef __attribute__((address_space(1))) T* GP;
+  return (T*)(GP)(((u64)hi << 32) | lo);
+}
+LCPC_DEV const u32* lane_at(const u32* base, u32 byte_off) { return reinterpret_cast<const u32*>(reinterpret_cast<const char*>(base) + byte_off); }
+LCPC_DEV u32* lane_at(u32* base, u32 byte_off) { return reinterpret_cast<u32*>(reinterpret_cast<char*>(base) + byte_off); }
 
 template <class FT, class C = u32> LCPC_DEV LN<FT::N> planes_get(const u32* base, C cnt, u32 e) {
   constexpr int N = FT::N;
@@ -101,6 +110,15 @@
     return planes_get<FT>(blk, NV * period, variant * period + jl);
   }
 }
+template <u32 NV> LCPC_DEV LN<9> pack_get_u(const u32* blk, u32 period, u32 uv, u32 lv, u32 jl) {
+  const u32 o16 = (lv * 2 * period + jl) << 4, o4 = (lv * period + jl) << 2;
+  const uint4 a = *reinterpret_cast<const uint4*>(lane_at(ubase(blk + (size_t)(uv * 2 + 0) * period * 4), o16));
+  const uint4 b = *reinterpret_cast<const uint4*>(lane_at(ubase(blk + (size_t)(uv * 2 + 1) * period * 4), o16));
+  const u32 c = *lane_at(ubase(blk + (size_t)NV * 2 * period * 4 + (size_t)uv * period), o4);
+  LN<9> t;
+  t.v[0] = a.x; t.v[1] = a.y; t.v[2] = a.z; t.v[3] = a.w; t.v[4] = b.x; t.v[5] = b.y; t.v[6] = b.z; t.v[7] = b.w; t.v[8] = c;
+  return t;
+}
 template <class FT, u32 NV> LCPC_DEV void pack_put(u32* blk, u32 period, u32 variant, u32 jl, const LN<FT::N>& x) {
   if constexpr (FT::N == 9) {
     *reinterpret_cast<uint4*>(blk + ((size_t)(variant * 2 + 0) * period + jl) * 4) = make_uint4(x.v[0], x.v[1], x.v[2], x.v[3]);
```

Measured after the change: 7.888 billion, median of 6. 1.1% higher.
